# jandrewrfarrell/RUFUS

Hardware: AMD Instinct MI355X
Metric: reads/sec through k-mer count+filter at k=25 (higher is better)
Workload: dtype u64; 1 GPU; synthetic 30x WGS trio (BASELINE configs[2]): genome 3100000000 bp, 620000000/620000000/620000000 x 150 bp reads per sample, on each of 1 GPU(s) 19 resident blocks of the subject (92 GB of packed reads in HBM, generated on the device in 2.9 s), 1000 SNVs, seed 12345, k=25, -s 8G -L 2, MinCov 5, MaxHashDepth 1200, MinQ 15, thresh 1; 2 minimizer-shard pass(es) per step (per-shard (pos,key)-sorted re; parallelism=read-block shard x1, mutant_kmers=24567, pulled_pairs=11560, passes=2, hbm_total=309220868096, hbm_free_at_start=308400881664, resident_read_bytes=92219805240, read_blocks=compact, run_map_budget_bytes=39836680704, checked=False, hbm_mapped_bytes=271656681472

## Files before the change

### include/rufus_hip.h

```cpp
#ifndef RUFUS_HIP_H
#define RUFUS_HIP_H

#include <stddef.h>
#include <stdint.h>

#ifdef __cplusplus
extern "C" {
#endif

#define RFX_OK 0
#define RFX_E_NODEVICE (-1)
#define RFX_E_INVAL (-2)
#define RFX_E_NOMEM (-3)
#define RFX_E_FULL (-4)
#define RFX_E_HIP (-5)
#define RFX_E_MIXEDCASE (-6)
#define RFX_E_RANGE (-7)
#define RFX_E_FORMAT (-8)

#define RFX_HISTO_BINS 10002

typedef struct rfx_ctx rfx_ctx;
typedef struct rfx_reads rfx_reads;
typedef struct rfx_table rfx_table;
// ... 140 lines not shown
int rfx_records_lsize(const rfx_records*);
int rfx_records_payload(const rfx_records*, void* out, size_t cap_bytes, int counter_len);
int rfx_records_payload_range(const rfx_records*, uint64_t first, uint64_t n, void* out, size_t cap_bytes,
                              int counter_len);
int rfx_records_get(const rfx_records*, uint64_t* keys, uint32_t* counts, uint64_t* pos);
rfx_records* rfx_records_load(rfx_ctx*, int k, int lsize, const uint64_t* cols, const void* payload, uint64_t n,
                              int counter_len);
rfx_records* rfx_records_load_fd(rfx_ctx*, int k, int lsize, const uint64_t* cols, int fd, uint64_t offset, uint64_t n,
                                 int counter_len);
rfx_records* rfx_records_from_dev(rfx_ctx*, int k, int lsize, const uint64_t* cols, const uint64_t* d_keys,
                                  const uint32_t* d_counts, uint64_t n);
const uint64_t* rfx_records_dev_keys(const rfx_records*);
const uint32_t* rfx_records_dev_counts(const rfx_records*);
const uint64_t* rfx_records_dev_pos(const rfx_records*);
int rfx_records_histo(const rfx_records*, uint64_t* histo );
int rfx_records_verify(const rfx_records*, uint32_t min_count, uint32_t max_count, uint64_t out[4]);
int rfx_records_checksum(const rfx_records*, uint64_t out[2]);
void rfx_records_free(rfx_records*);

int rfx_merge_unique(rfx_ctx*, const rfx_records* const* files, int n_files, uint32_t min_count, uint64_t* keys_out,
                     uint32_t* counts_out, uint64_t cap, uint64_t* n_out);
int rfx_query(const rfx_records* db, const uint64_t* keys, uint64_t n, uint32_t* counts_out);
int rfx_unique_to_subject(rfx_ctx*, const rfx_records* subject, const rfx_records* const* others, int n_others,
                          uint32_t min_count, uint32_t min_cov, uint32_t max_cov, uint64_t* keys_out,
                          uint32_t* counts_out, uint64_t cap, uint64_t* n_out);
rfx_records* rfx_records_subtract(rfx_ctx*, const rfx_records* a, const rfx_records* const* others, int n_others,
                                  uint32_t min_count, uint32_t max_count);

typedef struct rfx_binned rfx_binned;
typedef struct rfx_candidates rfx_candidates;
rfx_binned* rfx_count_finish_binned(rfx_table*, uint64_t lower, uint64_t upper, uint64_t* histo );
uint64_t rfx_binned_size(const rfx_binned*);
int rfx_binned_bits(const rfx_binned*);
void rfx_binned_free(rfx_binned*);
rfx_candidates* rfx_binned_strike(rfx_ctx*, rfx_binned* subject, const rfx_binned* control, uint32_t min_count,
                                  uint32_t max_count);
int rfx_candidates_strike(rfx_candidates*, const rfx_binned* control);
uint64_t rfx_candidates_size(const rfx_candidates*);
int rfx_candidates_get(const rfx_candidates*, uint64_t* keys_out);
void rfx_candidates_free(rfx_candidates*);

rfx_set* rfx_set_build(rfx_ctx*, const uint64_t* fwd_keys, uint64_t n, int k);
uint64_t rfx_set_size(const rfx_set*);
void rfx_set_free(rfx_set*);
int rfx_filter(rfx_set*, const rfx_reads*, int thresh, int last_base_skipped, uint32_t* hits_out,
               uint64_t* hitmask_out, uint64_t* n_hit_reads);
int rfx_filter_many(rfx_set*, const rfx_reads* const* blocks, int n, int thresh, int last_base_skipped,
                    uint64_t* const* hitmask_out, uint64_t* n_hit_reads);

typedef struct rfx_model_params {
  double sc, stdev, factor, skew, power;
} rfx_model_params;
int rfx_model_residuals(rfx_ctx*, const int64_t* histo, uint32_t n, const rfx_model_params* cand, int n_cand,
                        int log_resid, int inflection, int max_copy, double* resid_out);
int rfx_model_tables(rfx_ctx*, uint32_t n, const rfx_model_params* model, uint32_t* n_cols, double* dist,
                     size_t dist_cap, double* rowtot);

#define RFX_OVL_SAM 0
#define RFX_OVL_CONTIG 1
#define RFX_OVL_REGION 2
int rfx_overlap_score(rfx_ctx*, const char* a, int alen, const char* const* b, const int* blen, int nb, float min_pct,
                      int min_ovl, int variant, int* out );
typedef struct rfx_ovl_pool rfx_ovl_pool;
rfx_ovl_pool* rfx_ovl_pool_create(rfx_ctx*, const char* const* seqs, const int* lens, int n);
int rfx_ovl_pool_set(rfx_ovl_pool*, int idx, const char* seq, int len);
int rfx_ovl_pool_score(rfx_ovl_pool*, int query, const char* a_explicit, int a_len, const int* cand, int nb,
// ... 9 lines not shown
```

### profiles/summarize_pmc.py

```python
#!/usr/bin/env python3
import collections
import csv
import json
import re
import sys


NOT_CHAIN = frozenset((
    "k_synth_reads", "k_copy16",
    "k_flag_absent", "k_flag_absent_tiled", "k_fa_bounds", "k_flag_gather", "k_flag_range", "k_flag_rank", "k_flag_present",
    "k_compact_count", "k_compact_scatter", "k_scan_u64", "k_query", "k_strike_bins", "k_strike_cands",
    "k_filter", "k_filter_q", "k_filter_p", "k_filter_fast", "k_filter_big", "k_hits_mask", "k_mask_count", "k_set_bitmap",
    "k_set_bitmap_big", "k_set_bitmap_q", "k_set_bitmap_p",
    "k_set_insert", "k_set_bitmap_packed", "k_records_checksum", "k_records_verify", "k_check_sorted",
    "k_parse_records", "k_format_records", "k_txt_count", "k_txt_lines", "k_txt_reads", "k_txt_pack", "k_compute_pos", "k_annotate", "k_overlap_pool", "k_overlap_score",
    "k_model_colsum", "k_model_dist", "k_model_rowtot", "k_model_sum", "k_model_terms", "k_model_weights",
))
CHAIN_KNOWN = frozenset((
    "k_msp_part1", "k_msp_replay", "k_msp_count", "k_col_sums", "k_bin_group_sums", "k_bin_offsets", "k_scan_tail", "k_scan_sums",
    "k_scan_apply", "k_part2", "k_flag_if_gt", "k_slice_tag", "k_bin_hist", "k_bin_hist_stamp", "k_bin_hist_multi", "k_msp_leaf",
    "k_surv_place", "k_surv_hist", "k_surv_sort", "k_histo_bins", "k_histo_staged", "k_bin_count", "k_part1", "k_leaf", "k_leaf_compact", "k_bin_scatter",
    "k_tmp_start", "k_split_bins", "k_coarse_counts", "k_histo", "k_count_reads", "k_count_pairs", "k_table_pairs", "k_tile_count",
    "k_tile_scan", "k_tile_emit",
))


def kname(s):
    m = re.search(r"(k_[a-z0-9_]+|__amd_rocclr_[A-Za-z]+)", s)
    return m.group(1) if m else s[:40]


def load(path, counter):
    agg = collections.defaultdict(lambda: [0, 0.0])
    for r in csv.DictReader(open(path)):
        if r["Counter_Name"] == counter:
            a = agg[kname(r["Kernel_Name"])]
            a[0] += 1
            a[1] += float(r["Counter_Value"])
    return {k: (n, v / n) for k, (n, v) in agg.items()}


def main():
    f, w = load(sys.argv[1], "FETCH_SIZE"), load(sys.argv[2], "WRITE_SIZE")
    out = {}
# ... 33 lines not shown
```

### rufus_amd/capi.py

```python
from __future__ import annotations

import ctypes as C
import os
import sys

import numpy as np

_HERE = os.path.dirname(os.path.abspath(__file__))
LIB_PATH = os.environ.get("RFX_LIB") or os.path.join(_HERE, "librufus_hip.so")

HISTO_BINS = 10002
PACK_COUNT, PACK_FILTER = 1, 2
COUNT_AUTO, COUNT_TABLE, COUNT_P2L, COUNT_MSP = 0, 1, 2, 3
E_FULL, E_RANGE, E_MIXEDCASE = -4, -7, -6

u8p, u32p, u64p = C.POINTER(C.c_uint8), C.POINTER(C.c_uint32), C.POINTER(C.c_uint64)

SIGNATURES = {
    "rfx_version": (C.c_char_p, []),
    "rfx_strerror": (C.c_char_p, [C.c_int]),
    "rfx_last_error": (C.c_char_p, []),
    "rfx_jf_matrix": (C.c_int, [C.c_int, C.c_int, u64p]),
    "rfx_jf_pos": (C.c_uint64, [u64p, C.c_int, C.c_int, C.c_uint64]),
    "rfx_pack_words": (C.c_uint64, [u64p, C.c_uint32]),
    "rfx_pack_reads": (C.c_int, [C.c_char_p, C.c_char_p, u64p, C.c_uint32, C.c_int, C.c_int, u64p, u32p, u32p, u32p,
                                 u32p]),
    "rfx_pack_spans": (C.c_int, [C.c_void_p, u64p, u32p, u64p, C.c_uint32, C.c_int, C.c_int, u64p, u32p, u32p, u32p, u32p]),
    "rfx_hashlist_keys": (C.c_long, [C.c_char_p, C.c_size_t, C.c_int, C.c_int, u64p, C.c_size_t]),
    "rfx_jhash_header": (C.c_long, [C.c_int, C.c_int, u64p, C.c_int, C.c_int, C.c_int, C.POINTER(C.c_char_p),
                                    C.c_char_p, C.c_size_t]),
    "rfx_open": (C.c_void_p, [C.c_int, C.c_size_t]),
    "rfx_close": (None, [C.c_void_p]),
    "rfx_sync": (C.c_int, [C.c_void_p]),
    "rfx_host_alloc": (C.c_void_p, [C.c_size_t]),
    "rfx_host_alloc_lazy": (C.c_void_p, [C.c_size_t]),
    "rfx_host_pin": (C.c_int, [C.c_void_p]),
    "rfx_host_cpus": (C.c_uint, []),
    "rfx_host_free": (None, [C.c_void_p]),
    "rfx_stream": (C.c_void_p, [C.c_void_p]),
    "rfx_mem_stats": (C.c_int, [C.c_void_p, u64p, u64p, u64p]),
    "rfx_memcpy_dev": (C.c_int, [C.c_void_p, C.c_void_p, C.c_void_p, C.c_size_t]),
    "rfx_prof_enable": (C.c_int, [C.c_void_p, C.c_int]),
    "rfx_prof_filter": (C.c_int, [C.c_void_p, C.c_char_p]),
    "rfx_prof_reset": (C.c_int, [C.c_void_p]),
    "rfx_prof_query": (C.c_int, [C.c_void_p, C.c_char_p, C.POINTER(C.c_double), u64p]),
    "rfx_prof_names": (C.c_int, [C.c_void_p, C.c_char_p, C.c_size_t]),
    "rfx_reads_device_bytes": (C.c_uint64, [C.c_void_p]),
    "rfx_records_subtract": (C.c_void_p, [C.c_void_p, C.c_void_p, C.POINTER(C.c_void_p), C.c_int, C.c_uint32, C.c_uint32]),
    "rfx_count_finish_binned": (C.c_void_p, [C.c_void_p, C.c_uint64, C.c_uint64, u64p]),
    "rfx_binned_size": (C.c_uint64, [C.c_void_p]),
    "rfx_binned_bits": (C.c_int, [C.c_void_p]),
    "rfx_binned_free": (None, [C.c_void_p]),
    "rfx_binned_strike": (C.c_void_p, [C.c_void_p, C.c_void_p, C.c_void_p, C.c_uint32, C.c_uint32]),
    "rfx_candidates_strike": (C.c_int, [C.c_void_p, C.c_void_p]),
    "rfx_candidates_size": (C.c_uint64, [C.c_void_p]),
    "rfx_candidates_get": (C.c_int, [C.c_void_p, u64p]),
    "rfx_candidates_free": (None, [C.c_void_p]),
    "rfx_reads_upload": (C.c_void_p, [C.c_void_p, u64p, u32p, u32p, u32p, u32p, C.c_uint32]),
    "rfx_reads_free": (None, [C.c_void_p]),
    "rfx_reads_count": (C.c_uint32, [C.c_void_p]),
    "rfx_reads_bases": (C.c_uint64, [C.c_void_p]),
    "rfx_reads_words": (C.c_uint64, [C.c_void_p]),
    "rfx_reads_get": (C.c_int, [C.c_void_p, u64p, u32p, u32p, u32p, u32p]),
    "rfx_synth_reads": (C.c_void_p, [C.c_void_p, C.c_void_p, C.c_uint64, C.c_uint32, C.c_int, C.c_int]),
    "rfx_text_open": (C.c_void_p, [C.c_void_p, C.c_uint64]),
    "rfx_text_close": (None, [C.c_void_p]),
    "rfx_text_room": (C.c_uint64, [C.c_void_p]),
    "rfx_text_bytes": (C.c_uint64, [C.c_void_p]),
    "rfx_text_append": (C.c_long, [C.c_void_p, C.c_char_p, C.c_uint64]),
    "rfx_text_copied": (C.c_int, [C.c_void_p, C.c_long]),
    "rfx_text_wait": (C.c_int, [C.c_void_p, C.c_long]),
    "rfx_text_parse": (C.c_void_p, [C.c_void_p, C.c_int, C.c_int, C.POINTER(C.c_int)]),
    "rfx_text_fetch": (C.c_int, [C.c_void_p, C.c_char_p]),
    "rfx_text_reset": (None, [C.c_void_p]),
    "rfx_synth_text": (C.c_int, [C.c_void_p, C.c_uint64, C.c_uint32, C.c_void_p, C.c_void_p]),
    "rfx_synth_snv": (C.c_int, [C.c_void_p, C.c_uint32, u64p, C.c_char_p, C.c_char_p]),
    "rfx_synth_genome": (C.c_int, [C.c_void_p, C.c_uint64, C.c_uint64, C.c_void_p]),
    "rfx_count_begin": (C.c_void_p, [C.c_void_p, C.c_int, C.c_int, C.c_int, C.c_uint64, C.c_uint64, C.c_uint64]),
    "rfx_count_set_mode": (C.c_int, [C.c_void_p, C.c_int]),
    "rfx_count_set_passes": (C.c_int, [C.c_void_p, C.c_int]),
    "rfx_count_add": (C.c_int, [C.c_void_p, C.c_void_p]),
    "rfx_count_add_pairs_dev": (C.c_int, [C.c_void_p, C.c_void_p, C.c_void_p, C.c_uint64]),
    "rfx_count_stats": (C.c_int, [C.c_void_p, u64p, u64p, u64p]),
    "rfx_count_finish_begin": (C.c_void_p, [C.c_void_p, C.c_uint64, C.c_uint64, u64p]),
# ... 615 lines not shown
    while True:
        if _uniq_buf.get("cap") != cap or "k" not in _uniq_buf:
            _uniq_buf.update(cap=cap, k=np.zeros(cap, np.uint64), c=np.zeros(cap, np.uint32))
        keys, counts = _uniq_buf["k"], _uniq_buf["c"]
        n = C.c_uint64(0)
        rc = lib().rfx_unique_to_subject(ctx._h, subject._h, arr, len(others), min_count, min_cov, max_cov,
                                         _p(keys, u64p), _p(counts, u32p), cap, C.byref(n))
        if rc == E_RANGE and n.value > cap:
            cap = int(n.value)
            continue
        _check(rc, "rfx_unique_to_subject")
        return keys[:n.value].copy(), counts[:n.value].copy()


def records_subtract(ctx: Context, a: Records, others, min_count: int = 0, max_count: int = 0xFFFFFFFF) -> Records:
    arr = (C.c_void_p * max(1, len(others)))(*[f._h for f in others])
    return Records(ctx, lib().rfx_records_subtract(ctx._h, a._h, arr, len(others), min_count, max_count))


class Binned:

    def __init__(self, ctx: Context, handle):
        if not handle:
            raise RufusError("binned records: " + lib().rfx_last_error().decode())
        self.ctx, self._h = ctx, handle

    def __len__(self):
        return int(lib().rfx_binned_size(self._h))

    @property
    def bits(self):
        return lib().rfx_binned_bits(self._h)

    def free(self):
        if self._h:
            lib().rfx_binned_free(self._h)
            self._h = None


class Candidates:

    def __init__(self, ctx: Context, handle):
        if not handle:
            raise RufusError("candidates: " + lib().rfx_last_error().decode())
        self.ctx, self._h = ctx, handle

    def __len__(self):
        return int(lib().rfx_candidates_size(self._h))

    def strike(self, control: Binned):
        _check(lib().rfx_candidates_strike(self._h, control._h), "rfx_candidates_strike")

    def keys(self) -> np.ndarray:
        k = np.zeros(len(self), np.uint64)
        _check(lib().rfx_candidates_get(self._h, _p(k, u64p)), "rfx_candidates_get")
        return k[k != np.uint64(0xFFFFFFFFFFFFFFFF)]

    def free(self):
        if self._h:
            lib().rfx_candidates_free(self._h)
            self._h = None


def binned_strike(ctx: Context, subject: Binned, control, min_count: int = 0, max_count: int = 0xFFFFFFFF) -> Candidates:
    return Candidates(ctx, lib().rfx_binned_strike(ctx._h, subject._h, control._h if control is not None else None,
                                                   min_count, max_count))
# ... 78 lines not shown
```

### rufus_amd/csrc/rfx_api.hip

```cpp
#include <algorithm>
#include <condition_variable>
#include <mutex>
#include <cstdio>
#include <cstdlib>
#include <cstring>
#include <sys/mman.h>

#include <atomic>
#include <cerrno>
#include <chrono>
#include <queue>
#include <thread>
#include <vector>

#include <unistd.h>

#include "rfx_internal.h"

namespace {

thread_local char g_err[512] = "";

int hip_fail(hipError_t e, const char* what) {
  snprintf(g_err, sizeof g_err, "%s: %s", what, hipGetErrorString(e));
// ... 2805 lines not shown
      f.stage_extra += tail[2] + tail[2] / 4 + 64;
      msp_binned_drop(&f);
      continue;
    }
    rfx_binned* b = new rfx_binned();
    b->ctx = c;
    b->k = t->k;
    b->st = f.bstage;
    b->bin_at = f.bin_at;
    b->bin_lo = f.bin_lo;
    b->bin_hi = f.bin_hi;
    b->bits = f.bin_bits;
    b->n = total;
    f.bstage = rfxk::msp_stage{};
    f.bin_at = nullptr;
    msp_binned_drop(&f);
    if (histo) memcpy(histo, h.data(), RFX_HISTO_BINS * 8);
    if (kmers) {
      c->msp_surv_frac[lower >= 2 ? 1 : 0] = (double)total / (double)kmers;
      if (c->msp_surv_by_size.size() > 256) c->msp_surv_by_size.clear();
      c->msp_surv_by_size[msp_surv_key(lower, kmers)] = (double)total / (double)kmers;
    }
    uint64_t rec_bytes = 0;
    for (auto& sg : *t->segs) rec_bytes += sg.n * 8;
    if (rec_bytes > (4ull << 30)) p2l_drop_segments(t);
    return b;
  }
  snprintf(g_err, sizeof g_err, "MSP: the staging pool did not converge (internal error)");
  return nullptr;
}

uint64_t rfx_binned_size(const rfx_binned* b) { return b ? b->n : 0; }
int rfx_binned_bits(const rfx_binned* b) { return b ? b->bits : 0; }
void rfx_binned_free(rfx_binned* b) {
  if (!b) return;
  (void)hipSetDevice(b->ctx->device);
  leaf_stage_free(b->ctx, &b->st);
  dfree(b->ctx, b->bin_at);
  delete b;
}

rfx_candidates* rfx_binned_strike(rfx_ctx* c, rfx_binned* subject, const rfx_binned* control, uint32_t min_count,
                                  uint32_t max_count) {
  if (!c || !subject || subject->ctx != c || (control && (control->ctx != c || control->k != subject->k))) {
    snprintf(g_err, sizeof g_err, "rfx_binned_strike: bad argument");
    return nullptr;
  }
  (void)hipSetDevice(c->device);
  const rfxk::binned_view S = binned_view_of(subject), C = binned_view_of(control);
  uint64_t cap = std::max<uint64_t>(1u << 16, subject->n / 256);
  if (!control) cap = std::max<uint64_t>(cap, subject->n / 4);
  for (int attempt = 0; attempt < 2; ++attempt) {
    cap = std::min<uint64_t>(std::max<uint64_t>(cap, 1), 0xFFFFFFFFull);
    uint64_t* keys = (uint64_t*)dmalloc(c, cap * 8);
    uint32_t* bins = (uint32_t*)dmalloc(c, cap * 4);
    uint32_t* d_n = (uint32_t*)dmalloc(c, 4);
    auto drop = [&] { dfree(c, keys); dfree(c, bins); dfree(c, d_n); };
    if (!keys || !bins || !d_n) { drop(); snprintf(g_err, sizeof g_err, "rfx_binned_strike: out of device memory"); return nullptr; }
    hipError_t e = hipMemsetAsync(d_n, 0, 4, c->stream);
    uint32_t n = 0;
    if (e == hipSuccess) {
      rfxk::strike_bins(c, S, C, min_count, max_count, keys, bins, (uint32_t)cap, d_n);
      e = queue_read(c, &n, d_n, 4);
    }
    if (e == hipSuccess) e = ctx_sync(c);
    if (e != hipSuccess) { hip_fail(e, "rfx_binned_strike"); (void)ctx_sync(c); drop(); return nullptr; }
// ... 1387 lines not shown
```

### rufus_amd/csrc/rfx_msp.hip

```cpp
#include <algorithm>
#include <type_traits>

#include "rfx_devutil.h"
#include "rfx_internal.h"

#ifdef RFX_TIMING
__device__ unsigned long long g_tm[2048][32];
#define TM_ROW g_tm[blockIdx.x & 2047u]
#define TM_DECL unsigned long long tm_prev = __builtin_amdgcn_s_memtime()
#define TM(i) do { if (threadIdx.x == 0) { const unsigned long long tm_now = __builtin_amdgcn_s_memtime(); atomicAdd(&TM_ROW[i], tm_now - tm_prev); tm_prev = tm_now; } } while (0)
extern "C" int rfx_debug_timing(unsigned long long* out, int reset) {
  static unsigned long long h[2048][32];
  if (out) {
    if (hipMemcpyFromSymbol(h, HIP_SYMBOL(g_tm), sizeof(g_tm)) != hipSuccess) return -1;
    for (int i = 0; i < 32; ++i) {
      out[i] = 0;
      for (int w = 0; w < 2048; ++w) out[i] += h[w][i];
    }
  }
  if (reset) {
    void* p = nullptr;
    if (hipGetSymbolAddress(&p, HIP_SYMBOL(g_tm)) != hipSuccess || hipMemset(p, 0, sizeof(g_tm)) != hipSuccess) return -1;
  }
  return 0;
// ... 1310 lines not shown
    if (end > o) fn((size_t)ch * v.chunk, o, end);
    if (last) break;
    ch = v.fill[v.n_chunks + ch];
    o = 0;
  }
}
template <class F>
__device__ __forceinline__ void binned_segments(const rfxk::binned_view& v, uint32_t gbin, F&& fn) {
  binned_segments(v, binned_marks(v, gbin), fn);
}
template <class F>
__device__ __forceinline__ void binned_range(const rfxk::binned_view& v, uint32_t b0, uint32_t b1, const uint4 first, F&& fn) {
  for (uint32_t b = b0; b < b1; ++b)
    binned_segments(v, b == b0 ? first : binned_marks(v, b), [&](size_t f0, uint32_t o, uint32_t e) { fn(b, f0, o, e); });
}

__device__ __forceinline__ void cand_append(bool surv, uint64_t key, uint32_t bin, uint64_t* __restrict__ out_k,
                                            uint32_t* __restrict__ out_b, uint32_t cap, uint32_t* __restrict__ out_n) {
  const unsigned long long m = __ballot(surv);
  if (!m) return;
  const uint32_t lane = threadIdx.x & 63u, leader = (uint32_t)__ffsll(m) - 1u;
  uint32_t base = 0;
  if (lane == leader) base = atomicAdd(out_n, (uint32_t)__popcll(m));
  base = __shfl(base, (int)leader, 64);
  if (surv) {
    const uint32_t at = base + (uint32_t)__popcll(m & ((1ull << lane) - 1ull));
    if (at < cap) {
      out_k[at] = key;
      out_b[at] = bin;
    }
  }
}

constexpr int SB_BLK = 128, SB_SET_LOG2 = 11, SB_SET = 1 << SB_SET_LOG2, SB_TILE = SB_SET / 2;
__device__ __forceinline__ uint32_t sb_hash(uint64_t key) { return (uint32_t)((key * 0x9E3779B97F4A7C15ull) >> 40); }

__global__ __launch_bounds__(SB_BLK) void k_strike_bins(const rfxk::binned_view S, const rfxk::binned_view C, int ubits, uint32_t u_lo,
                                                        uint32_t u_hi, uint32_t lo, uint32_t hi, uint64_t* __restrict__ out_k,
                                                        uint32_t* __restrict__ out_b, uint32_t cap, uint32_t* __restrict__ out_n) {
  __shared__ unsigned long long s_set[SB_SET];
  const int ds = S.bits - ubits, dc = C.bin_at ? C.bits - ubits : 0;
  for (uint32_t u = u_lo + blockIdx.x; u < u_hi; u += gridDim.x) {
    uint32_t n_s = 0, n_c = 0;
    const uint32_t s0 = u << ds, s1 = (u + 1u) << ds, c0 = u << dc, c1 = C.bin_at ? (u + 1u) << dc : c0;
    const uint4 ms = binned_marks(S, s0), mc = binned_marks(C, c0);
    binned_range(S, s0, s1, ms, [&](uint32_t, size_t, uint32_t o, uint32_t e) { n_s += e - o; });
    if (!n_s) continue;
    binned_range(C, c0, c1, mc, [&](uint32_t, size_t, uint32_t o, uint32_t e) { n_c += e - o; });
    const uint32_t tiles = n_c ? (n_c + SB_TILE - 1u) / SB_TILE : 1u;
    const bool single = tiles == 1u;
    for (uint32_t t = 0; t < tiles; ++t) {
      const uint32_t t0 = t * SB_TILE, t1 = min(t0 + (uint32_t)SB_TILE, n_c);
      uint32_t lg = 8;
      while ((1u << lg) < 2u * (t1 - t0)) ++lg;
      const uint32_t mask = (1u << lg) - 1u;
      for (uint32_t i = threadIdx.x; i <= mask; i += SB_BLK) s_set[i] = RFX_EMPTY;
      __syncthreads();
      if (t1 > t0) {
        uint32_t idx0 = 0;
        binned_range(C, c0, c1, mc, [&](uint32_t, size_t first, uint32_t o, uint32_t e) {
            const uint32_t from = max(idx0, t0), to = min(idx0 + (e - o), t1);
            for (uint32_t i = from + threadIdx.x; i < to; i += SB_BLK) {
              const unsigned long long key = C.keys[first + o + (i - idx0)];
              uint32_t h = sb_hash(key) & mask;
              for (;;) {
                const unsigned long long old = atomicCAS(&s_set[h], (unsigned long long)RFX_EMPTY, key);
                if (old == RFX_EMPTY || old == key) break;
                h = (h + 1u) & mask;
              }
            }
            idx0 += e - o;
          });
      }
      __syncthreads();
      binned_range(S, s0, s1, ms, [&](uint32_t b, size_t first, uint32_t o, uint32_t e) {
          for (uint32_t i0 = o; i0 < e; i0 += SB_BLK) {
            const uint32_t i = i0 + threadIdx.x;
            uint64_t key = 0;
            uint32_t c = 0;
            if (i < e) {
              c = S.counts[first + i];
              key = S.keys[first + i];
              bool drop = false;
              if (t == 0 && c && (c < lo || c > hi)) drop = true;
              if (c && !drop && t1 > t0) {
                uint32_t h = sb_hash(key) & mask;
                for (;;) {
                  const unsigned long long v = s_set[h];
                  if (v == key) drop = true;
                  if (v == key || v == RFX_EMPTY) break;
                  h = (h + 1u) & mask;
                }
              }
              if (drop) {
                c = 0;
                if (!single) S.counts[first + i] = 0;
              }
            }
            if (single) cand_append(c != 0, key, b, out_k, out_b, cap, out_n);
          }
        });
      __syncthreads();
    }
    if (!single)
      binned_range(S, s0, s1, ms, [&](uint32_t b, size_t first, uint32_t o, uint32_t e) {
          for (uint32_t i0 = o; i0 < e; i0 += SB_BLK) {
            const uint32_t i = i0 + threadIdx.x;
            const bool live = i < e && S.counts[first + i] != 0;
            cand_append(live, live ? S.keys[first + i] : 0ull, b, out_k, out_b, cap, out_n);
          }
        });
  }
}

__global__ __launch_bounds__(256) void k_strike_cands(uint64_t* __restrict__ keys, const uint32_t* __restrict__ bins, uint32_t n,
                                                      int bits, const rfxk::binned_view C) {
  const uint32_t lane = threadIdx.x & 63u, wave = (blockIdx.x * 256u + threadIdx.x) >> 6, n_waves = gridDim.x * 4u;
  for (uint32_t i = wave; i < n; i += n_waves) {
    const uint64_t key = keys[i];
    if (key == RFX_EMPTY) continue;
    const uint32_t sb = bins[i];
    const uint32_t b0 = C.bits >= bits ? sb << (C.bits - bits) : sb >> (bits - C.bits);
    const uint32_t b1 = C.bits >= bits ? (sb + 1u) << (C.bits - bits) : b0 + 1u;
    bool found = false;
    for (uint32_t b = b0; b < b1; ++b)
      binned_segments(C, b, [&](size_t first, uint32_t o, uint32_t e) {
        for (uint32_t j = o + lane; j < e; j += 64u) found |= C.keys[first + j] == key;
      });
    if (__ballot(found) && lane == 0) keys[i] = RFX_EMPTY;
  }
}

__global__ __launch_bounds__(256) void k_histo_staged(const uint32_t* __restrict__ counts, const uint32_t* __restrict__ fill,
                                                       const uint32_t* __restrict__ more, uint32_t CH, uint32_t n_chunks,
                                                       unsigned long long* __restrict__ g_histo,
                                                       unsigned long long* __restrict__ g_total) {
  __shared__ uint32_t s_h[RFX_HISTO_BINS];
  for (int i = threadIdx.x; i < RFX_HISTO_BINS; i += 256) s_h[i] = 0;
  __syncthreads();
  const uint32_t n_used = min(*more, n_chunks);
  unsigned long long total = 0;
  for (uint32_t ch = blockIdx.x; ch < n_used; ch += gridDim.x) {
    const uint32_t n = min(fill[ch], CH);
    const uint32_t* const src = counts + (size_t)ch * CH;
// ... 120 lines not shown
                     inst0, bs0, seg_ext, ext0, P, k, lower, upper, st.keys, st.counts, st.chunk, st.fill, more,           \
                     st.n_chunks, flag, err, stage_short, force_mixed, bin_at)
    if (canonical) {
      if (geo) RFX_MSP_LEAF(true, 1);
      else RFX_MSP_LEAF(true, 0);
    } else {
      if (geo) RFX_MSP_LEAF(false, 1);
      else RFX_MSP_LEAF(false, 0);
    }
#undef RFX_MSP_LEAF
  }
  if (!bin_at) {
    rfx_span sp(c, "k_surv_place");
    const uint32_t pg = std::min<uint32_t>(st.n_chunks, (uint32_t)c->n_cu * (uint32_t)std::max(1, 160 * 1024 / (16 * 1024 + SP_N * 12 + 2048)));
    hipLaunchKernelGGL(k_surv_place, dim3(pg), dim3(SP_BLK), 0, c->stream, st.keys, st.counts, st.chunk, st.fill, more, grid,
                       st.n_chunks, lut, ntab, sel_bits, shift1, pos_lo, pos_hi, out_w, out_c, cur, cap, flag);
  }
}

uint32_t msp_leaf_chunk_room(int geo, uint32_t chunk) { return chunk - MSP_LEAF_PASS_MAX(geo); }
uint32_t msp_leaf_chunk_kept(uint32_t chunk) { return chunk >= 16384u ? 65536u : chunk; }

void histo_staged(rfx_ctx* c, const msp_stage& st, unsigned long long* d_histo, unsigned long long* d_total) {
  rfx_span sp(c, "k_histo");
  const uint32_t grid = std::max<uint32_t>(1, std::min<uint32_t>(st.n_chunks, (uint32_t)c->n_cu * 4));
  hipLaunchKernelGGL(k_histo_staged, dim3(grid), dim3(256), 0, c->stream, st.counts, st.fill, st.more, st.chunk, st.n_chunks,
                     d_histo, d_total);
}

void strike_bins(rfx_ctx* c, const binned_view& S, const binned_view& C, uint32_t lo, uint32_t hi, uint64_t* out_k,
                 uint32_t* out_b, uint32_t cap, uint32_t* out_n) {
  rfx_span sp(c, "k_strike_bins");
  const int ubits = C.bin_at ? std::min(S.bits, C.bits) : S.bits;
  const int ds = S.bits - ubits;
  const uint32_t u_lo = S.bin_lo >> ds, u_hi = (uint32_t)((((uint64_t)S.bin_hi + (1u << ds) - 1)) >> ds);
  if (u_hi <= u_lo) return;
  const uint32_t grid = std::min<uint32_t>(u_hi - u_lo, (uint32_t)c->n_cu * 10);
  hipLaunchKernelGGL(k_strike_bins, dim3(grid), dim3(SB_BLK), 0, c->stream, S, C, ubits, u_lo, u_hi, lo, hi, out_k, out_b, cap,
                     out_n);
}

void strike_cands(rfx_ctx* c, uint64_t* keys, const uint32_t* bins, uint32_t n, int bits, const binned_view& C) {
  if (!n) return;
  rfx_span sp(c, "k_strike_cands");
  const uint32_t grid = std::min<uint32_t>((n + 3) / 4, (uint32_t)c->n_cu * 8);
  hipLaunchKernelGGL(k_strike_cands, dim3(grid), dim3(256), 0, c->stream, keys, bins, n, bits, C);
}

void surv_hist(rfx_ctx* c, const uint64_t* buf_a, const uint32_t* coarse_cur, uint32_t cap_a, uint32_t P2, int shift2,
               uint64_t* fine_tot, int rec_mode, int k, uint64_t n_hint) {
  rfx_span sp(c, rec_mode ? "k_rec_hist" : "k_surv_hist");
  uint32_t W = 8;
  if (n_hint > (1ull << 27)) W = (uint32_t)c->n_cu * 2 / P1_BINS * 4;
#define RFX_SH(MODE)                                                                                                \
  hipLaunchKernelGGL(k_surv_hist<MODE>, dim3(P1_BINS * W), dim3(L2_BLOCK), 0, c->stream, buf_a, coarse_cur, cap_a, P2, \
                     shift2, W, k, (unsigned long long*)fine_tot)
  if (rec_mode == 0) RFX_SH(0);
  else if (rec_mode == 1) RFX_SH(1);
  else RFX_SH(2);
#undef RFX_SH
}

void flag_if_gt(rfx_ctx* c, const uint64_t* d_value, uint64_t limit, unsigned int* d_flag) {
  hipLaunchKernelGGL(k_flag_if_gt, dim3(1), dim3(1), 0, c->stream, d_value, limit, d_flag);
}

void histo_bins(rfx_ctx* c, const uint32_t* counts, const uint32_t* coarse_cur, uint32_t cap,
                unsigned long long* d_histo) {
  rfx_span sp(c, "k_histo");
  const uint32_t W = 16;
  hipLaunchKernelGGL(k_histo_bins, dim3(P1_BINS * W), dim3(256), 0, c->stream, counts, coarse_cur, cap, W, d_histo);
}
// ... 12 lines not shown
```

Before: 1.111 billion reads/s.

## Restructure strike kernel to per-wave hash sets with register-prefetched bins and slow fallback

```diff
diff --git a/include/rufus_hip.h b/include/rufus_hip.h
--- a/include/rufus_hip.h
+++ b/include/rufus_hip.h
@@ -196,6 +196,7 @@
 rfx_binned* rfx_count_finish_binned(rfx_table*, uint64_t lower, uint64_t upper, uint64_t* histo );
 uint64_t rfx_binned_size(const rfx_binned*);
 int rfx_binned_bits(const rfx_binned*);
+uint64_t rfx_binned_largest_bin(const rfx_binned*);
 void rfx_binned_free(rfx_binned*);
 rfx_candidates* rfx_binned_strike(rfx_ctx*, rfx_binned* subject, const rfx_binned* control, uint32_t min_count,
                                   uint32_t max_count);
diff --git a/profiles/summarize_pmc.py b/profiles/summarize_pmc.py
--- a/profiles/summarize_pmc.py
+++ b/profiles/summarize_pmc.py
@@ -9,7 +9,7 @@
 NOT_CHAIN = frozenset((
     "k_synth_reads", "k_copy16",
     "k_flag_absent", "k_flag_absent_tiled", "k_fa_bounds", "k_flag_gather", "k_flag_range", "k_flag_rank", "k_flag_present",
-    "k_compact_count", "k_compact_scatter", "k_scan_u64", "k_query", "k_strike_bins", "k_strike_cands",
+    "k_compact_count", "k_compact_scatter", "k_scan_u64", "k_query", "k_strike_bins", "k_strike_slow", "k_strike_cands",
     "k_filter", "k_filter_q", "k_filter_p", "k_filter_fast", "k_filter_big", "k_hits_mask", "k_mask_count", "k_set_bitmap",
     "k_set_bitmap_big", "k_set_bitmap_q", "k_set_bitmap_p",
     "k_set_insert", "k_set_bitmap_packed", "k_records_checksum", "k_records_verify", "k_check_sorted",
diff --git a/rufus_amd/capi.py b/rufus_amd/capi.py
--- a/rufus_amd/capi.py
+++ b/rufus_amd/capi.py
@@ -50,6 +50,7 @@
     "rfx_count_finish_binned": (C.c_void_p, [C.c_void_p, C.c_uint64, C.c_uint64, u64p]),
     "rfx_binned_size": (C.c_uint64, [C.c_void_p]),
     "rfx_binned_bits": (C.c_int, [C.c_void_p]),
+    "rfx_binned_largest_bin": (C.c_uint64, [C.c_void_p]),
     "rfx_binned_free": (None, [C.c_void_p]),
     "rfx_binned_strike": (C.c_void_p, [C.c_void_p, C.c_void_p, C.c_void_p, C.c_uint32, C.c_uint32]),
     "rfx_candidates_strike": (C.c_int, [C.c_void_p, C.c_void_p]),
@@ -731,6 +732,9 @@
     def bits(self):
         return lib().rfx_binned_bits(self._h)
 
+    def largest_bin(self) -> int:
+        return int(lib().rfx_binned_largest_bin(self._h))
+
     def free(self):
         if self._h:
             lib().rfx_binned_free(self._h)
diff --git a/rufus_amd/csrc/rfx_api.hip b/rufus_amd/csrc/rfx_api.hip
--- a/rufus_amd/csrc/rfx_api.hip
+++ b/rufus_amd/csrc/rfx_api.hip
@@ -2861,6 +2861,35 @@
 
 uint64_t rfx_binned_size(const rfx_binned* b) { return b ? b->n : 0; }
 int rfx_binned_bits(const rfx_binned* b) { return b ? b->bits : 0; }
+uint64_t rfx_binned_largest_bin(const rfx_binned* b) {
+  if (!b || !b->bin_at || b->bin_hi <= b->bin_lo) return 0;
+  rfx_ctx* c = b->ctx;
+  (void)hipSetDevice(c->device);
+  const uint32_t nb = b->bin_hi - b->bin_lo, nc = b->st.n_chunks, CH = b->st.chunk;
+  std::vector<uint2> at((size_t)nb * 2);
+  std::vector<uint32_t> fill((size_t)nc * 2);
+  hipError_t e = queue_read(c, at.data(), b->bin_at, at.size() * sizeof(uint2));
+  if (e == hipSuccess && nc) e = queue_read(c, fill.data(), b->st.fill, fill.size() * 4);
+  if (e == hipSuccess) e = ctx_sync(c);
+  if (e != hipSuccess) { hip_fail(e, "rfx_binned_largest_bin"); (void)ctx_sync(c); return 0; }
+  uint64_t best = 0;
+  for (uint32_t i = 0; i < nb; ++i) {
+    const uint2 a = at[2 * (size_t)i], z = at[2 * (size_t)i + 1];
+    if (z.x >= nc) continue;
+    uint64_t n = 0;
+    uint32_t ch = a.x, o = a.y;
+    for (uint32_t hops = 0; hops <= nc && ch < nc; ++hops) {
+      const bool last = ch == z.x;
+      const uint32_t end = std::min(last ? z.y : fill[ch], CH);
+      if (end > o) n += end - o;
+      if (last) break;
+      ch = fill[nc + ch];
+      o = 0;
+    }
+    best = std::max(best, n);
+  }
+  return best;
+}
 void rfx_binned_free(rfx_binned* b) {
   if (!b) return;
   (void)hipSetDevice(b->ctx->device);
diff --git a/rufus_amd/csrc/rfx_msp.hip b/rufus_amd/csrc/rfx_msp.hip
--- a/rufus_amd/csrc/rfx_msp.hip
+++ b/rufus_amd/csrc/rfx_msp.hip
@@ -1366,84 +1366,304 @@
   }
 }
 
-constexpr int SB_BLK = 128, SB_SET_LOG2 = 11, SB_SET = 1 << SB_SET_LOG2, SB_TILE = SB_SET / 2;
+constexpr int SB_BLK = 256, SB_WAVES = SB_BLK / 64, SB_SET_LOG2 = 10, SB_SET = 1 << SB_SET_LOG2, SB_TILE = SB_SET / 2;
+constexpr int SB_FAST = SB_SET * 3 / 4;
+constexpr int SB_REG = 8;
 __device__ __forceinline__ uint32_t sb_hash(uint64_t key) { return (uint32_t)((key * 0x9E3779B97F4A7C15ull) >> 40); }
-
-__global__ __launch_bounds__(SB_BLK) void k_strike_bins(const rfxk::binned_view S, const rfxk::binned_view C, int ubits, uint32_t u_lo,
+__device__ __forceinline__ uint32_t sb_lane(uint32_t v, uint32_t l) {
+  return (uint32_t)__builtin_amdgcn_readlane((int)v, (int)l);
+}
+__device__ __forceinline__ void sb_wave_sync() {
+  __builtin_amdgcn_fence(__ATOMIC_ACQ_REL, "wavefront");
+  __builtin_amdgcn_wave_barrier();
+}
+
+template <int NB>
+struct sb_side {
+  uint32_t p[NB + 1];
+  uint64_t adj[NB];
+  bool ok;
+};
+template <int NB>
+__device__ __forceinline__ sb_side<NB> sb_describe(const rfxk::binned_view& v, const uint4 m, uint32_t j) {
+  sb_side<NB> d;
+  d.ok = true;
+  uint32_t n = 0;
+#pragma unroll
+  for (int q = 0; q < NB; ++q) {
+    const uint32_t l = j * NB + q;
+    const uint32_t ax = sb_lane(m.x, l), ay = sb_lane(m.y, l), ex = sb_lane(m.z, l), ey = sb_lane(m.w, l);
+    uint32_t len = 0;
+    if (ax < v.n_chunks && ex < v.n_chunks) {
+      const uint32_t end = min(ey, v.chunk);
+      if (ax != ex) d.ok = false;
+      else if (end > ay) len = end - ay;
+    }
+    d.p[q] = n;
+    d.adj[q] = (uint64_t)ax * v.chunk + ay - n;
+    n += len;
+  }
+  d.p[NB] = n;
+  return d;
+}
+template <int NB>
+__device__ __forceinline__ uint64_t sb_at(const sb_side<NB>& d, uint32_t i) {
+  uint64_t a = d.adj[0];
+#pragma unroll
+  for (int q = 1; q < NB; ++q)
+    if (i >= d.p[q]) a = d.adj[q];
+  return a + i;
+}
+template <int NB>
+__device__ __forceinline__ uint32_t sb_bin(const sb_side<NB>& d, uint32_t i) {
+  uint32_t b = 0;
+#pragma unroll
+  for (int q = 1; q < NB; ++q) b += i >= d.p[q];
+  return b;
+}
+
+__device__ __forceinline__ uint32_t sb_insert(unsigned long long* set, uint32_t mask, unsigned long long key) {
+  uint32_t h = sb_hash(key) & mask;
+  for (;;) {
+    const unsigned long long old = atomicCAS(&set[h], (unsigned long long)RFX_EMPTY, key);
+    if (old == RFX_EMPTY || old == key) return h;
+    h = (h + 1u) & mask;
+  }
+}
+__device__ __forceinline__ bool sb_holds(const unsigned long long* set, uint32_t mask, unsigned long long key) {
+  uint32_t h = sb_hash(key) & mask;
+  for (;;) {
+    const unsigned long long v = set[h];
+    if (v == key) return true;
+    if (v == RFX_EMPTY) return false;
+    h = (h + 1u) & mask;
+  }
+}
+
+template <int NBS, int NBC>
+__device__ __forceinline__ bool sb_is_slow(const sb_side<NBS>& s, const sb_side<NBC>& c) {
+  return !s.ok || !c.ok || (s.p[NBS] != 0 && c.p[NBC] > (uint32_t)SB_FAST);
+}
+
+__device__ __forceinline__ void sb_unit_slow(const rfxk::binned_view& S, const rfxk::binned_view& C, unsigned long long* set,
+                                          uint32_t u, int ds, int dc, uint32_t lo, uint32_t hi, uint64_t* __restrict__ out_k,
+                                          uint32_t* __restrict__ out_b, uint32_t cap, uint32_t* __restrict__ out_n) {
+  const uint32_t lane = threadIdx.x & 63u;
+  uint32_t n_s = 0, n_c = 0;
+  const uint32_t s0 = u << ds, s1 = (u + 1u) << ds, c0 = u << dc, c1 = C.bin_at ? (u + 1u) << dc : c0;
+  const uint4 ms = binned_marks(S, s0), mc = binned_marks(C, c0);
+  binned_range(S, s0, s1, ms, [&](uint32_t, size_t, uint32_t o, uint32_t e) { n_s += e - o; });
+  if (!n_s) return;
+  binned_range(C, c0, c1, mc, [&](uint32_t, size_t, uint32_t o, uint32_t e) { n_c += e - o; });
+  const uint32_t tiles = n_c ? (n_c + SB_TILE - 1u) / SB_TILE : 1u;
+  const bool single = tiles == 1u;
+  for (uint32_t t = 0; t < tiles; ++t) {
+    const uint32_t t0 = t * SB_TILE, t1 = min(t0 + (uint32_t)SB_TILE, n_c);
+    uint32_t lg = 8;
+    while ((1u << lg) < 2u * (t1 - t0)) ++lg;
+    const uint32_t mask = (1u << lg) - 1u;
+    if (t1 > t0) {
+      uint32_t idx0 = 0;
+      binned_range(C, c0, c1, mc, [&](uint32_t, size_t first, uint32_t o, uint32_t e) {
+          const uint32_t from = max(idx0, t0), to = min(idx0 + (e - o), t1);
+          for (uint32_t i = from + lane; i < to; i += 64u) sb_insert(set, mask, C.keys[first + o + (i - idx0)]);
+          idx0 += e - o;
+        });
+    }
+    sb_wave_sync();
+    binned_range(S, s0, s1, ms, [&](uint32_t b, size_t first, uint32_t o, uint32_t e) {
+        for (uint32_t i0 = o; i0 < e; i0 += 64u) {
+          const uint32_t i = i0 + lane;
+          uint64_t key = 0;
+          uint32_t c = 0;
+          if (i < e) {
+            c = S.counts[first + i];
+            key = S.keys[first + i];
+            bool drop = false;
+            if (t == 0 && c && (c < lo || c > hi)) drop = true;
+            if (c && !drop && t1 > t0) drop = sb_holds(set, mask, key);
+            if (drop) {
+              c = 0;
+              if (!single) S.counts[first + i] = 0;
+            }
+          }
+          if (single) cand_append(c != 0, key, b, out_k, out_b, cap, out_n);
+        }
+      });
+    sb_wave_sync();
+    for (uint32_t i = lane; i <= mask; i += 64u) set[i] = RFX_EMPTY;
+    sb_wave_sync();
+  }
+  if (!single)
+    binned_range(S, s0, s1, ms, [&](uint32_t b, size_t first, uint32_t o, uint32_t e) {
+        for (uint32_t i0 = o; i0 < e; i0 += 64u) {
+          const uint32_t i = i0 + lane;
+          const bool live = i < e && S.counts[first + i] != 0;
+          cand_append(live, live ? S.keys[first + i] : 0ull, b, out_k, out_b, cap, out_n);
+        }
+      });
+}
+
+template <int NBS, int NBC>
+__global__ __launch_bounds__(SB_BLK) void k_strike_bins(const rfxk::binned_view S, const rfxk::binned_view C, uint32_t u_lo,
                                                         uint32_t u_hi, uint32_t lo, uint32_t hi, uint64_t* __restrict__ out_k,
                                                         uint32_t* __restrict__ out_b, uint32_t cap, uint32_t* __restrict__ out_n) {
-  __shared__ unsigned long long s_set[SB_SET];
-  const int ds = S.bits - ubits, dc = C.bin_at ? C.bits - ubits : 0;
-  for (uint32_t u = u_lo + blockIdx.x; u < u_hi; u += gridDim.x) {
-    uint32_t n_s = 0, n_c = 0;
-    const uint32_t s0 = u << ds, s1 = (u + 1u) << ds, c0 = u << dc, c1 = C.bin_at ? (u + 1u) << dc : c0;
-    const uint4 ms = binned_marks(S, s0), mc = binned_marks(C, c0);
-    binned_range(S, s0, s1, ms, [&](uint32_t, size_t, uint32_t o, uint32_t e) { n_s += e - o; });
-    if (!n_s) continue;
-    binned_range(C, c0, c1, mc, [&](uint32_t, size_t, uint32_t o, uint32_t e) { n_c += e - o; });
-    const uint32_t tiles = n_c ? (n_c + SB_TILE - 1u) / SB_TILE : 1u;
-    const bool single = tiles == 1u;
-    for (uint32_t t = 0; t < tiles; ++t) {
-      const uint32_t t0 = t * SB_TILE, t1 = min(t0 + (uint32_t)SB_TILE, n_c);
-      uint32_t lg = 8;
-      while ((1u << lg) < 2u * (t1 - t0)) ++lg;
-      const uint32_t mask = (1u << lg) - 1u;
-      for (uint32_t i = threadIdx.x; i <= mask; i += SB_BLK) s_set[i] = RFX_EMPTY;
-      __syncthreads();
-      if (t1 > t0) {
-        uint32_t idx0 = 0;
-        binned_range(C, c0, c1, mc, [&](uint32_t, size_t first, uint32_t o, uint32_t e) {
-            const uint32_t from = max(idx0, t0), to = min(idx0 + (e - o), t1);
-            for (uint32_t i = from + threadIdx.x; i < to; i += SB_BLK) {
-              const unsigned long long key = C.keys[first + o + (i - idx0)];
-              uint32_t h = sb_hash(key) & mask;
-              for (;;) {
-                const unsigned long long old = atomicCAS(&s_set[h], (unsigned long long)RFX_EMPTY, key);
-                if (old == RFX_EMPTY || old == key) break;
-                h = (h + 1u) & mask;
-              }
-            }
-            idx0 += e - o;
-          });
-      }
-      __syncthreads();
-      binned_range(S, s0, s1, ms, [&](uint32_t b, size_t first, uint32_t o, uint32_t e) {
-          for (uint32_t i0 = o; i0 < e; i0 += SB_BLK) {
-            const uint32_t i = i0 + threadIdx.x;
-            uint64_t key = 0;
-            uint32_t c = 0;
-            if (i < e) {
-              c = S.counts[first + i];
-              key = S.keys[first + i];
-              bool drop = false;
-              if (t == 0 && c && (c < lo || c > hi)) drop = true;
-              if (c && !drop && t1 > t0) {
-                uint32_t h = sb_hash(key) & mask;
-                for (;;) {
-                  const unsigned long long v = s_set[h];
-                  if (v == key) drop = true;
-                  if (v == key || v == RFX_EMPTY) break;
-                  h = (h + 1u) & mask;
-                }
-              }
-              if (drop) {
-                c = 0;
-                if (!single) S.counts[first + i] = 0;
-              }
-            }
-            if (single) cand_append(c != 0, key, b, out_k, out_b, cap, out_n);
-          }
-        });
-      __syncthreads();
-    }
-    if (!single)
-      binned_range(S, s0, s1, ms, [&](uint32_t b, size_t first, uint32_t o, uint32_t e) {
-          for (uint32_t i0 = o; i0 < e; i0 += SB_BLK) {
-            const uint32_t i = i0 + threadIdx.x;
-            const bool live = i < e && S.counts[first + i] != 0;
-            cand_append(live, live ? S.keys[first + i] : 0ull, b, out_k, out_b, cap, out_n);
-          }
-        });
+  static_assert(NBS == 1 || NBC == 1, "one side's bin is the unit");
+  static_assert(SB_FAST % 64 == 0 && SB_FAST / 64 <= 16 && SB_FAST >= SB_REG * 64, "slots remembered two to a register");
+  constexpr uint32_t UB = 64 / (NBS > NBC ? NBS : NBC), MASK = SB_SET - 1;
+  constexpr int CR = SB_FAST / 64;
+  __shared__ unsigned long long s_sets[SB_WAVES][SB_SET];
+  const uint32_t lane = threadIdx.x & 63u, wv = (uint32_t)__builtin_amdgcn_readfirstlane((int)(threadIdx.x >> 6));
+  unsigned long long* const set = s_sets[wv];
+  const uint32_t n_waves = gridDim.x * SB_WAVES, n_blocks = (u_hi - u_lo + UB - 1u) / UB;
+  for (uint32_t i = lane; i < (uint32_t)SB_SET; i += 64u) set[i] = RFX_EMPTY;
+  sb_wave_sync();
+
+  struct unit_t {
+    sb_side<NBS> s;
+    sb_side<NBC> c;
+    uint32_t u, n_s, n_c;
+    bool slow;
+  };
+  struct tile_t {
+    uint64_t sk[SB_REG], ck[SB_REG];
+    uint32_t sc[SB_REG];
+  };
+  const uint4 ones = make_uint4(~0u, ~0u, ~0u, ~0u);
+  auto marks_of = [&](const rfxk::binned_view& v, uint32_t blk, uint32_t nb) {
+    return lane < UB * nb ? binned_marks(v, (u_lo + blk * UB) * nb + lane) : ones;
+  };
+  auto describe = [&](const uint4 ms, const uint4 mc, uint32_t blk, uint32_t j) {
+    unit_t d;
+    d.u = u_lo + blk * UB + j;
+    d.s = sb_describe<NBS>(S, ms, j);
+    d.c = sb_describe<NBC>(C, mc, j);
+    const bool in = d.u < u_hi;
+    d.slow = in && sb_is_slow<NBS, NBC>(d.s, d.c);
+    d.n_s = in && !d.slow ? d.s.p[NBS] : 0u;
+    d.n_c = d.n_s ? d.c.p[NBC] : 0u;
+    return d;
+  };
+  auto fetch = [&](const unit_t& d, tile_t& t) {
+#pragma unroll
+    for (int r = 0; r < SB_REG; ++r) {
+      const uint32_t i = lane + 64u * (uint32_t)r;
+      t.sk[r] = 0;
+      t.sc[r] = 0;
+      if (i < d.n_s) {
+        const uint64_t a = sb_at<NBS>(d.s, i);
+        t.sk[r] = S.keys[a];
+        t.sc[r] = S.counts[a];
+      }
+    }
+#pragma unroll
+    for (int r = 0; r < SB_REG; ++r) {
+      const uint32_t i = lane + 64u * (uint32_t)r;
+      t.ck[r] = 0;
+      if (i < d.n_c) t.ck[r] = C.keys[sb_at<NBC>(d.c, i)];
+    }
+  };
+  auto process = [&](const unit_t& d, const tile_t& t) {
+    if (!d.n_s) return;
+    uint32_t slots[(CR + 1) / 2];
+#pragma unroll
+    for (int r = 0; r < (CR + 1) / 2; ++r) slots[r] = 0;
+    if (d.n_c) {
+#pragma unroll
+      for (int r = 0; r < CR; ++r) {
+        const uint32_t i = lane + 64u * (uint32_t)r;
+        if (64u * (uint32_t)r < d.n_c) {
+          if (i < d.n_c) {
+            const unsigned long long key = r < SB_REG ? t.ck[r < SB_REG ? r : 0] : C.keys[sb_at<NBC>(d.c, i)];
+            slots[r >> 1] |= sb_insert(set, MASK, key) << (16 * (r & 1));
+          }
+        }
+      }
+      sb_wave_sync();
+    }
+    auto one = [&](uint32_t i, uint64_t key, uint32_t c) {
+      bool cand = i < d.n_s && c != 0 && c >= lo && c <= hi;
+      if (cand && d.n_c) cand = !sb_holds(set, MASK, key);
+      cand_append(cand, key, (d.u * NBS) + sb_bin<NBS>(d.s, i), out_k, out_b, cap, out_n);
+    };
+#pragma unroll
+    for (int r = 0; r < SB_REG; ++r)
+      if (64u * (uint32_t)r < d.n_s) one(lane + 64u * (uint32_t)r, t.sk[r], t.sc[r]);
+    for (uint32_t i0 = 64u * SB_REG; i0 < d.n_s; i0 += 64u) {
+      const uint32_t i = i0 + lane;
+      uint64_t key = 0;
+      uint32_t c = 0;
+      if (i < d.n_s) {
+        const uint64_t a = sb_at<NBS>(d.s, i);
+        key = S.keys[a];
+        c = S.counts[a];
+      }
+      one(i, key, c);
+    }
+    if (d.n_c) {
+      sb_wave_sync();
+#pragma unroll
+      for (int r = 0; r < CR; ++r)
+        if (lane + 64u * (uint32_t)r < d.n_c) set[(slots[r >> 1] >> (16 * (r & 1))) & 0xFFFFu] = RFX_EMPTY;
+      sb_wave_sync();
+    }
+  };
+
+  uint32_t blk = blockIdx.x * SB_WAVES + wv;
+  if (blk >= n_blocks) return;
+  uint4 ms = marks_of(S, blk, NBS), mc = marks_of(C, blk, NBC);
+  unit_t nx = describe(ms, mc, blk, 0);
+  tile_t nt;
+  fetch(nx, nt);
+  for (;;) {
+    const uint32_t nblk = blk + n_waves;
+    const bool more = nblk < n_blocks;
+    uint4 ms_n = ones, mc_n = ones;
+    if (more) {
+      ms_n = marks_of(S, nblk, NBS);
+      mc_n = marks_of(C, nblk, NBC);
+    }
+#pragma unroll 1
+    for (uint32_t j = 0; j < UB; ++j) {
+      const unit_t cu = nx;
+      const tile_t ct = nt;
+      nx = j + 1u < UB ? describe(ms, mc, blk, j + 1u) : describe(ms_n, mc_n, nblk, 0);
+      fetch(nx, nt);
+      process(cu, ct);
+    }
+    if (!more) break;
+    ms = ms_n;
+    mc = mc_n;
+    blk = nblk;
+  }
+}
+
+template <int NBS, int NBC>
+__global__ __launch_bounds__(SB_BLK) void k_strike_slow(const rfxk::binned_view S, const rfxk::binned_view C, uint32_t u_lo,
+                                                        uint32_t u_hi, uint32_t lo, uint32_t hi, uint64_t* __restrict__ out_k,
+                                                        uint32_t* __restrict__ out_b, uint32_t cap, uint32_t* __restrict__ out_n,
+                                                        int ds, int dc, int all_slow) {
+  constexpr uint32_t UB = 64 / (NBS > NBC ? NBS : NBC);
+  __shared__ unsigned long long s_sets[SB_WAVES][SB_SET];
+  const uint32_t lane = threadIdx.x & 63u, wv = (uint32_t)__builtin_amdgcn_readfirstlane((int)(threadIdx.x >> 6));
+  unsigned long long* const set = s_sets[wv];
+  const uint32_t n_waves = gridDim.x * SB_WAVES, n_blocks = (u_hi - u_lo + UB - 1u) / UB;
+  for (uint32_t i = lane; i < (uint32_t)SB_SET; i += 64u) set[i] = RFX_EMPTY;
+  sb_wave_sync();
+  const uint4 ones = make_uint4(~0u, ~0u, ~0u, ~0u);
+  for (uint32_t blk = blockIdx.x * SB_WAVES + wv; blk < n_blocks; blk += n_waves) {
+    uint4 ms = ones, mc = ones;
+    if (!all_slow) {
+      if (lane < UB * NBS) ms = binned_marks(S, (u_lo + blk * UB) * NBS + lane);
+      if (lane < UB * NBC) mc = binned_marks(C, (u_lo + blk * UB) * NBC + lane);
+    }
+#pragma unroll 1
+    for (uint32_t j = 0; j < UB; ++j) {
+      const uint32_t u = u_lo + blk * UB + j;
+      if (u >= u_hi) break;
+      if (!all_slow && !sb_is_slow<NBS, NBC>(sb_describe<NBS>(S, ms, j), sb_describe<NBC>(C, mc, j))) continue;
+      sb_unit_slow(S, C, set, u, ds, dc, lo, hi, out_k, out_b, cap, out_n);
+    }
   }
 }
 
@@ -1630,12 +1850,25 @@
                  uint32_t* out_b, uint32_t cap, uint32_t* out_n) {
   rfx_span sp(c, "k_strike_bins");
   const int ubits = C.bin_at ? std::min(S.bits, C.bits) : S.bits;
-  const int ds = S.bits - ubits;
+  const int ds = S.bits - ubits, dc = C.bin_at ? C.bits - ubits : 0, d = std::max(ds, dc);
   const uint32_t u_lo = S.bin_lo >> ds, u_hi = (uint32_t)((((uint64_t)S.bin_hi + (1u << ds) - 1)) >> ds);
   if (u_hi <= u_lo) return;
-  const uint32_t grid = std::min<uint32_t>(u_hi - u_lo, (uint32_t)c->n_cu * 10);
-  hipLaunchKernelGGL(k_strike_bins, dim3(grid), dim3(SB_BLK), 0, c->stream, S, C, ubits, u_lo, u_hi, lo, hi, out_k, out_b, cap,
-                     out_n);
+  const int all_slow = d > 1 || getenv("RFX_STRIKE_SLOW") != nullptr;
+  const uint32_t per_block = all_slow ? 64u : 64u >> d, n_blocks = (u_hi - u_lo + per_block - 1) / per_block;
+  const uint32_t wgs = (n_blocks + SB_WAVES - 1) / SB_WAVES;
+  const uint32_t grid = std::min<uint32_t>(wgs, (uint32_t)c->n_cu * 3), grid_slow = std::min<uint32_t>(wgs, (uint32_t)c->n_cu * 4);
+#define RFX_STRIKE(NBS, NBC)                                                                                               \
+  do {                                                                                                                     \
+    if (!all_slow)                                                                                                         \
+      hipLaunchKernelGGL((k_strike_bins<NBS, NBC>), dim3(grid), dim3(SB_BLK), 0, c->stream, S, C, u_lo, u_hi, lo, hi, out_k, \
+                         out_b, cap, out_n);                                                                               \
+    hipLaunchKernelGGL((k_strike_slow<NBS, NBC>), dim3(grid_slow), dim3(SB_BLK), 0, c->stream, S, C, u_lo, u_hi, lo, hi,    \
+                       out_k, out_b, cap, out_n, ds, dc, all_slow);                                                        \
+  } while (0)
+  if (all_slow || d == 0) RFX_STRIKE(1, 1);
+  else if (ds == 1) RFX_STRIKE(2, 1);
+  else RFX_STRIKE(1, 2);
+#undef RFX_STRIKE
 }
 
 void strike_cands(rfx_ctx* c, uint64_t* keys, const uint32_t* bins, uint32_t n, int bits, const binned_view& C) {
```

Result: no change. 1.117 billion reads/s (median of 6 runs) (+0.5%).
